# De-Rosa/PPO-BipedalWalker

Measured on NVIDIA B200. Metric: walker env-steps/sec (SAT physics step), higher is better.
Workload: dtype f32

## Files before the change

### ppo-bipedalwalker_b200/csrc/physics_lanes.cu

```cuda
#include <cstdio>
#include <cstdlib>
#include "physics.cuh"
#include "physics_math.cuh"

#ifndef WB_SAT_UNROLL
#define WB_SAT_UNROLL 6
#endif
#ifndef WB_BODY_SLOT
#define WB_BODY_SLOT 0
#endif

namespace wb {
namespace pl {
constexpr int kSatUnroll = WB_SAT_UNROLL;

constexpr unsigned kFull = 0xFFFFFFFFu;

#ifdef WB_PHASE_PROFILE
__device__ unsigned long long g_prof[24];
__device__ __forceinline__ long long prof_clock() {
  long long t;
  asm volatile("mov.u64 %0, %%clock64;" : "=l"(t)::"memory");
  return t;
}
__device__ long long g_prof_sat_scratch;
#endif


__constant__ Material c_materials[WB_MAX_MATERIALS];
__constant__ float c_init_state[kStateFloats];
__constant__ FloorConst c_floor;

enum { LLL = 0, LLU = 1, BODY = 2, RLL = 3, RLU = 4, FLOOR = 5 };

constexpr int kV2Cen = 30;
constexpr int kV2Vel = 35;
constexpr int kV2Count = 40;
constexpr int kFOmega = 0;
constexpr int kFAngle = 5;
constexpr int kFCount = 10;

__device__ __forceinline__ int nverts(int b) { return b == BODY ? 5 : 6; }

template <int L_, int E_>
struct Env {
  static constexpr int L = L_;
  static constexpr int E = E_;
  float2* v2;
  float* f;
  const FloorConst* fl;
  int sub;
  int gsub;
  int gshift;
  int col;
  bool live;
  int flags;
  float im_w;
  float ii_pole;
  float e_ww, mu_ww, e_wf, mu_wf;
};

template <class EV> __device__ __forceinline__ float2& V2(const EV& e, int slot) { return e.v2[slot * EV::E]; }
template <class EV> __device__ __forceinline__ float& F1(const EV& e, int slot) { return e.f[slot * EV::E]; }
template <class EV> __device__ __forceinline__ float inv_inertia(const EV& e, int b) { return b == BODY ? 0.0003f : e.ii_pole; }
template <class EV> __device__ __forceinline__ void set_materials(EV& e, const Material& mw, const Material& mf) {
  e.im_w = mw.inverse_mass;
  e.ii_pole = fmul(0.001f, mw.inverse_mass);
  e.e_ww = net_max(mw.restitution, mw.restitution);
  e.mu_ww = net_min(mw.friction, mw.friction);
  e.e_wf = net_max(mw.restitution, mf.restitution);
  e.mu_wf = net_min(mw.friction, mf.friction);
}
template <int L> __device__ __forceinline__ void lanes_sync() { if (L > 1) __syncwarp(); }
template <class EV, int G> __device__ __forceinline__ bool group_any(const EV& e, bool pred) {
  if (EV::L == 1) return pred;
  const unsigned b = __ballot_sync(kFull, pred);
  return ((b >> e.gshift) & ((1u << G) - 1u)) != 0u;
}

struct BodyDyn {
  float2 c, v;
  float w, im, ii;
};

template <class EV> __device__ __forceinline__ BodyDyn load_dyn(const EV& e, int b) {
  BodyDyn d;
  d.c = V2(e, kV2Cen + b);
  d.v = V2(e, kV2Vel + b);
  d.w = F1(e, kFOmega + b);
  d.im = e.im_w;
  d.ii = inv_inertia(e, b);
  return d;
}
template <class EV> __device__ __forceinline__ BodyDyn floor_dyn(const EV& e) {
  BodyDyn d;
  d.c = e.fl->cen;
  d.v = mk2(0.0f, 0.0f);
  d.w = 0.0f;
  d.im = 0.0f;
  d.ii = 0.0f;
  return d;
}
template <class EV> __device__ __forceinline__ void store_dyn(const EV& e, int b, const BodyDyn& d) {
  V2(e, kV2Vel + b) = d.v;
  F1(e, kFOmega + b) = d.w;
}

__device__ __forceinline__ void calculate_impulse(const BodyDyn& A, const BodyDyn& B, float2 contact, float force, float2 n,
                                                  float2& rA, float2& rB, float& impulse) {
  rA = vsub(contact, A.c);
  const float2 perpA = mk2(-rA.y, rA.x);
  const float kA = vdot(n, perpA);
  rB = vsub(contact, B.c);
  const float2 perpB = mk2(-rB.y, rB.x);
  const float kB = vdot(n, perpB);
  const float2 va = vadd(A.v, vmul(perpA, A.w));
  const float2 vb = vadd(B.v, vmul(perpB, B.w));
  const float2 vrel = vsub(vb, va);
  const float vn = vdot(vrel, n);
  const float j = fmul(-force, vn);
  const float2 k = mk2(kA, kB);
  const float2 kki = vmul2_nosum(vmul2_nosum(k, k), mk2(A.ii, B.ii));
  const float denom = fadd(fadd(fadd(A.im, B.im), kki.x), kki.y);
  impulse = fdiv(j, denom);
}

__device__ __forceinline__ void apply_impulses(BodyDyn& A, BodyDyn& B, float2 n, float impulse, float2 rA, float2 rB) {
  const float2 J = vmul(n, impulse);
  const float2 velA = vsub(A.v, vmul(J, A.im));
  const float2 velB = vadd(B.v, vmul(J, B.im));
  const float2 perpA = mk2(-rA.y, rA.x);
  const float wA = fsub(A.w, fmul(vdot(perpA, J), A.ii));
  const float2 perpB = mk2(-rB.y, rB.x);
  const float wB = fadd(B.w, fmul(vdot(perpB, J), B.ii));
  A.v = velA;
  B.v = velB;
  A.w = wA;
  B.w = wB;
}

template <class EV, int G>
__device__ __forceinline__ void move_bodies(const EV& e, bool on, int A, float2 dA, bool moveB, int B, float2 dB) {
#pragma unroll
  for (int it0 = 0; it0 < 14; it0 += G) {
    const int it = it0 + e.gsub;
    const bool second = it >= 7;
    const int k = second ? it - 7 : it;
    const int b = second ? B : A;
    if (on && it < 14 && (!second || moveB)) {
      const int slot = (k < 6) ? b * 6 + k : kV2Cen + b;
      V2(e, slot) = vadd(V2(e, slot), second ? dB : dA);
    }
  }
}

template <class EV, bool TRACE, int G = EV::L>
__device__ __forceinline__ void joint_step(const EV& e, int A, int ia, int B, int ib, wb_joint_trace* tr) {
  const bool leader = (G == EV::L) ? e.sub == 0 : e.gsub == 0;
  const float2 pA = V2(e, A * 6 + ia);
  const float2 pB = V2(e, B * 6 + ib);
  float2 ab = vsub(pB, pA);
  const float depth = fsqrt(vdot(ab, ab));
  if (TRACE) {
    if (tr && e.live && leader) {
      tr->active = !(depth < 0.1f);
      tr->depth = depth;
    }
  }
  const bool active = e.live && !(depth < 0.1f);
  if (!__any_sync(kFull, active)) return;
  ab = vnormalize_fast(ab);
  const float2 dA = vhalf(vmul(ab, depth));
  const float2 dB = vhalf(vmul(vneg(ab), depth));
  BodyDyn X = load_dyn(e, B);
  BodyDyn Y = load_dyn(e, A);
  lanes_sync<EV::L>();
  move_bodies<EV, G>(e, active, A, dA, true, B, dB);
  X.c = vadd(X.c, dB);
// ... 463 lines not shown
            rec.c1y = c1.y;
          }
        }
      }
      const float2 dA = FLOORB ? vmul(normal, depth) : vhalf(vmul(normal, depth));
      const float2 dB = FLOORB ? mk2(0.f, 0.f) : vhalf(vmul(vneg(normal), depth));
      lanes_sync<EV::L>();
      move_bodies<EV, G>(e, colliding, A, dA, !FLOORB, B, dB);
      X.c = vadd(X.c, dA);
      if (!FLOORB) Y.c = vadd(Y.c, dB);
      if (G == 1) {
        if (ncp > 0) resolve_impulses(X, Y, ncp, c0, c1, normal, FLOORB ? e.e_wf : e.e_ww, FLOORB ? e.mu_wf : e.mu_ww);
      } else {
        resolve_impulses_split(X, Y, ncp, c0, c1, normal, FLOORB ? e.e_wf : e.e_ww, FLOORB ? e.mu_wf : e.mu_ww, (e.gsub & 1) != 0);
      }
      if (ncp > 0 && colliding && e.gsub == 0) {
        store_dyn(e, A, X);
        if (!FLOORB) store_dyn(e, B, Y);
      }
      lanes_sync<EV::L>();
    }
  }
  if (TRACE) {
    if (tr && want && e.gsub == 0) *tr = rec;
  }
#ifdef WB_PHASE_PROFILE
  const unsigned prof_want = __ballot_sync(kFull, want), prof_coll = __ballot_sync(kFull, colliding);
  if (!TRACE && (threadIdx.x & 31) == 0) {
    const long long rp_t2 = prof_clock();
    const int k = FLOORB ? 1 : 0;
    atomicAdd(&g_prof[8 + 4 * k + 0], (unsigned long long)(rp_t1 - rp_t0));
    atomicAdd(&g_prof[8 + 4 * k + 1], (unsigned long long)(rp_t2 - rp_t1));
    atomicAdd(&g_prof[8 + 4 * k + 2], 1ull);
    atomicAdd(&g_prof[8 + 4 * k + 3], (unsigned long long)__popc(prof_want) | ((unsigned long long)__popc(prof_coll) << 32));
  }
#endif
}


template <class EV, int R>
__device__ __forceinline__ void integrate_step(const EV& e, bool on, int b, int q, int nq, float dt, float2 (&P)[R]) {
  float2 v = V2(e, kV2Vel + b);
  v = vadd(v, vmul(mk2(0.0f, 980.0f), dt));
  const float2 d = vmul(v, dt);
  const float w = F1(e, kFOmega + b);
  const float theta = fmul(w, dt);
  float ang = fadd(F1(e, kFAngle + b), theta);
  const float PI_F = 3.14159274f, TAU_F = 6.28318548f;
  if (ang > PI_F) ang = fsub(ang, TAU_F);
  else if (ang < -PI_F) ang = fadd(ang, TAU_F);
  float m11, m12;
  rotz(theta, m11, m12);
  const float2 cen = vadd(V2(e, kV2Cen + b), d);
  lanes_sync<EV::L>();
#pragma unroll
  for (int r = 0; r < R; r++) {
    const int i = r * nq + q;
    P[r] = mk2(0.0f, 0.0f);
    if (i < 6 && on) {
      float2 p = vadd(V2(e, b * 6 + i), d);
      p = vsub(p, cen);
      const float2 t = vrotate(p, m11, m12);
      P[r] = vadd(t, cen);
      V2(e, b * 6 + i) = P[r];
    }
  }
  if (q == 0 && on) {
    V2(e, kV2Cen + b) = cen;
    V2(e, kV2Vel + b) = v;
    F1(e, kFAngle + b) = ang;
  }
  lanes_sync<EV::L>();
}

template <class EV, int G, bool TRACE>
__device__ __forceinline__ void resolve_candidates(EV& e, bool on, int b, wb_pair_trace* tr_base) {
  const int slot = (0x75420 >> (4 * b)) & 0xF;
  const int partner = (0x34F01 >> (4 * b)) & 0xF;
  const bool floor_first = (e.flags & WB_FLAG_FLOOR_FIRST) != 0;
#pragma unroll 1
  for (int phase = 0; phase < 3; phase++) {
    if (phase == 1) {
      const bool want = on && b != BODY;
      if (__any_sync(kFull, want))
        resolve_pair<EV, G, TRACE, false>(e, want, b, b == BODY ? LLL : partner, (TRACE && tr_base) ? tr_base + slot + (floor_first ? 1 : 0) : nullptr);
    } else {
      const bool want = on && ((b == BODY) ? (phase == 0) : ((phase == 0) == floor_first));
      if (__any_sync(kFull, want))
        resolve_pair<EV, G, TRACE, true>(e, want, b, FLOOR, (TRACE && tr_base) ? tr_base + slot + ((b == BODY || floor_first) ? 0 : 1) : nullptr);
    }
  }
}

template <class EV, int G, bool TRACE>
__device__ __forceinline__ void body_step(EV& e, bool on, int b, float dt, wb_pair_trace* tr_base) {
  float2 P[(6 + G - 1) / G];
  integrate_step(e, on, b, e.gsub, G, dt, P);
  resolve_candidates<EV, G, TRACE>(e, on, b, tr_base);
}

template <class EV, int G, bool TRACE>
__device__ __forceinline__ void legs_sweep(EV& e, bool left, float dt, wb_pair_trace* tr_base) {
  static_assert(G >= 4, "two or more lanes per body in slot 0");
  constexpr int H = G / 2;
  constexpr int R = (6 + H - 1) / H;
  const int base = e.gshift - (left ? 0 : G);
#pragma unroll 1
  for (int k = 0; k < 2; k++) {
    const bool body_lane = k == 0 && left && e.gsub >= H;
    const int seg = left ? (k == 0 ? LLL : LLU) : (k == 0 ? RLL : RLU);
    float2 P[R];
    integrate_step(e, e.live, body_lane ? BODY : seg, body_lane ? e.gsub - H : e.gsub, (k == 0 && left) ? H : G, dt, P);
    if (k == 0) {
      float2 Q[6];
#pragma unroll
      for (int i = 0; i < 6; i++) {
        Q[i].x = __shfl_sync(kFull, P[i / H].x, base + H + i % H);
        Q[i].y = __shfl_sync(kFull, P[i / H].y, base + H + i % H);
      }
      float2 mn, mx;
      aabb6(Q, mn, mx);
      const unsigned hits = __ballot_sync(kFull, body_lane && e.live && aabb_hit(mn, mx, e.fl->bb_min, e.fl->bb_max));
      const bool body_hit = ((hits >> base) & ((1u << G) - 1u)) != 0u;
      if (body_hit) e.flags |= 1 << BODY;
      wb_pair_trace* tr = (TRACE && tr_base) ? tr_base + 4 : nullptr;
      if (TRACE) {
        if (tr && e.live && left && e.gsub == 0 && !body_hit) *tr = pair_trace_no_sat(FLOOR, false);
      }
      if (hits != 0u) resolve_pair<EV, G, TRACE, true, -1, true>(e, left && body_hit, left ? BODY : RLL, FLOOR, tr);
    }
    resolve_candidates<EV, G, TRACE>(e, e.live, seg, tr_base);
  }
}

template <class EV>
__device__ __forceinline__ void store_observation(const EV& e, float* dst) {
  const float2 j0 = V2(e, BODY * 6 + 1), j2 = V2(e, LLU * 6 + 2), j3 = V2(e, RLU * 6 + 2), bv = V2(e, kV2Vel + BODY);
  float4* d4 = reinterpret_cast<float4*>(dst);
  d4[0] = make_float4(fdiv(j0.x, 900.0f), fdiv(j0.y, 500.0f), fdiv(j2.x, 900.0f), fdiv(j2.y, 500.0f));
  d4[1] = make_float4(fdiv(j3.x, 900.0f), fdiv(j3.y, 500.0f), fdiv(bv.x, 60.0f), fdiv(bv.y, 60.0f));
  d4[2] = make_float4(F1(e, kFAngle + LLL), F1(e, kFAngle + LLU), F1(e, kFAngle + RLL), F1(e, kFAngle + RLU));
}

template <int E>
__device__ __forceinline__ int record_word(int f) {
  if (f < 58) {
    const int vtx = f >> 1, slot = vtx + (vtx >= 17 ? 1 : 0);
    return slot * E * 2 + (f & 1);
  }
  if (f < 78) return (kV2Cen + ((f - 58) >> 1)) * E * 2 + (f & 1);
  return kV2Count * E * 2 + (f - 78) * E;
}

template <int L, int LEGS, bool TRACE>
__global__ void __launch_bounds__(32, (L <= 4 || L == 16) ? 16 : 8) physics_lanes_kernel(const PhysicsParams p) {
  static_assert(LEGS == 1 || (LEGS == 2 && L >= 2), "the leg split needs at least two lanes per environment");
  constexpr int E = 32 / L;
  __shared__ __align__(16) float s_state[(kV2Count * 2 + kFCount) * E];
  __shared__ FloorConst s_floor;
  const int lane = threadIdx.x;
  const int env0 = blockIdx.x * E;

  for (int w = lane; w < (int)(sizeof(FloorConst) / 4); w += 32)
    reinterpret_cast<uint32_t*>(&s_floor)[w] = reinterpret_cast<const uint32_t*>(&c_floor)[w];
  for (int idx = lane; idx < 88 * E; idx += 32) {
    int f, c;
    if (idx < 78 * E) {
      const int slot = idx / (2 * E), r = idx % (2 * E);
      c = r >> 1;
      f = 2 * slot + (r & 1);
    } else {
      f = 78 + (idx - 78 * E) / E;
      c = idx % E;
    }
    const int env = env0 + c;
    const float v = (env < p.n) ? p.state[state_index(f, env, p.n_pad)] : c_init_state[f];
    s_state[record_word<E>(f) + (f < 78 ? 2 * c : c)] = v;
  }
  __syncwarp();

  using EV = Env<L, E>;
  EV e;
  const int col = lane / L;
  const int env = env0 + col;
  e.v2 = reinterpret_cast<float2*>(s_state) + col;
  e.f = s_state + kV2Count * E * 2 + col;
  e.fl = &s_floor;
  e.sub = lane % L;
  e.gsub = e.sub;
  e.gshift = col * L;
  e.live = env < p.n;
  const int envc = e.live ? env : 0;
  if (e.sub == 0) V2(e, BODY * 6 + 5) = V2(e, BODY * 6);
  float* torque_rows = p.state + (size_t)88 * p.n_pad + envc;

  e.flags = p.flags[envc];
  int steps = p.steps[envc];
  {
    const Material mw = c_materials[p.walker_mat[envc]];
    const Material mf = c_materials[p.floor_mat[envc]];
    set_materials(e, mw, mf);
  }
  float2 pos = mk2(p.pos[envc], p.pos[p.n_pad + envc]);
  __syncwarp();

  auto write_initial_record = [&](bool on) {
    if (!__any_sync(kFull, on)) return;
    __syncwarp();
    if (on && e.sub == 0) {
#pragma unroll 1
      for (int f = 0; f < 88; f++) s_state[record_word<E>(f) + (f < 78 ? 2 * col : col)] = c_init_state[f];
      V2(e, BODY * 6 + 5) = V2(e, BODY * 6);
      for (int k = 0; k < 4; k++) torque_rows[(size_t)k * p.n_pad] = c_init_state[88 + k];
    }
    __syncwarp();
  };

  if (p.phases & kPhaseResetMasked) {
    const bool on = e.live && (p.reset_mask == nullptr || p.reset_mask[envc]);
    write_initial_record(on);
    if (on) {
      e.flags = (p.phases & kPhaseFirstEpisode) ? 0 : WB_FLAG_FLOOR_FIRST;
      steps = 0;
      pos = V2(e, kV2Cen + BODY);
    }
  }
  if (p.phases & kPhaseIncSteps) steps++;

  if (p.phases & kPhaseTakeActions) {
    if (e.live && e.sub == 0) {
      const float4 a4 = *reinterpret_cast<const float4*>(p.actions + (size_t)env * 4);
      const float act[4] = {a4.x, a4.y, a4.z, a4.w};
#pragma unroll
      for (int k = 0; k < 4; k++) {
        float a = act[k];
        if (a >= 1.0f) a = 1.0f;
        else if (a <= -1.0f) a = -1.0f;
        const float change = fsub(a, torque_rows[(size_t)k * p.n_pad]);
        torque_rows[(size_t)k * p.n_pad] = a;
        const int bodyB = (k == 0) ? LLU : (k == 1) ? RLU : (k == 2) ? LLL : RLL;
        F1(e, kFOmega + bodyB) = fadd(F1(e, kFOmega + bodyB), fmul(change, 5.0f));
      }
    }
    __syncwarp();
  }

  if (p.phases & kPhaseStepObjects) {
    const float dt = fdiv(p.dt, (float)p.iterations);
#pragma unroll 1
    for (int it = 0; it < p.iterations; it++) {
      wb_joint_trace* jt = nullptr;
      wb_pair_trace* pt = nullptr;
      if (TRACE) {
        if (p.joint_trace) jt = p.joint_trace + ((size_t)envc * p.iterations + it) * 4;
        if (p.pair_trace) pt = p.pair_trace + ((size_t)envc * p.iterations + it) * WB_PAIR_SLOTS;
      }
      if (LEGS == 1) {
#pragma unroll 1
        for (int k = 0; k < 4; k++) {
          const int A = (0x4122 >> (4 * k)) & 0xF, B = (0x3041 >> (4 * k)) & 0xF;
          joint_step<EV, TRACE>(e, A, k < 2 ? 1 : 2, B, k < 2 ? 4 : 3, jt ? jt + k : nullptr);
        }
      } else {
        constexpr int G = L / LEGS;
        joint_step<EV, TRACE>(e, BODY, 1, LLU, 4, jt ? jt + 0 : nullptr);
        const int leg = e.sub / G;
        e.gsub = e.sub % G;
        e.gshift = col * L + leg * G;
        const bool left = leg == 0;
        joint_step<EV, TRACE, G>(e, left ? LLU : BODY, left ? 2 : 1, left ? LLL : RLU, left ? 3 : 4, jt ? jt + (left ? 2 : 1) : nullptr);
        e.gsub = e.sub;
        e.gshift = col * L;
        joint_step<EV, TRACE>(e, RLU, 2, RLL, 3, jt ? jt + 3 : nullptr);
      }
      if (LEGS == 1) {
#pragma unroll 1
        for (int b = 0; b < 5; b++) body_step<EV, L, TRACE>(e, e.live, b, dt, pt);
      } else {
        constexpr int G = L / LEGS;
        const int leg = e.sub / G;
        e.gsub = e.sub % G;
        e.gshift = col * L + leg * G;
        if constexpr (G >= 4 && !WB_BODY_SLOT) {
          legs_sweep<EV, G, TRACE>(e, leg == 0, dt, pt);
        } else {
#pragma unroll 1
          for (int k = 0; k < 3; k++) {
            const bool on = e.live && (leg == 0 || k < 2);
            body_step<EV, G, TRACE>(e, on, leg == 0 ? k : (k < 2 ? RLL + k : RLU), dt, pt);
          }
        }
        e.gsub = e.sub;
        e.gshift = col * L;
      }
    }
    if (LEGS == 2) e.flags |= __shfl_xor_sync(kFull, e.flags, L / LEGS);
  }

  if (p.phases & kPhaseObserve) {
    const float2 prev = pos;
    pos = V2(e, kV2Cen + BODY);
    if (e.flags & ((1 << BODY) | (1 << LLU) | (1 << RLU))) e.flags |= WB_FLAG_TERMINAL;
    const float dx = fsub(pos.x, prev.x);
    const float h = fdiv(V2(e, BODY * 6 + 1).y, 500.0f);
    float r = 0.0f;
    r = fadd(r, (dx > 0.0f && h < 1.6f) ? dx : 0.0f);
    r = fsub(r, (h > 1.65f) ? -0.1f : 0.0f);
    bool terminal = false;
    if ((e.flags & WB_FLAG_TERMINAL) || steps > p.max_timesteps) {
      if (e.flags & WB_FLAG_TERMINAL) r = fsub(r, 40.0f);
      terminal = true;
    }
    if (pos.x > 900.0f) {
      r = fadd(r, 80.0f);
      terminal = true;
    }
    const bool reset_now = e.live && terminal && (p.phases & kPhaseAutoReset);
    write_initial_record(reset_now);
    if (reset_now) {
      e.flags = WB_FLAG_FLOOR_FIRST;
      steps = 0;
      pos = V2(e, kV2Cen + BODY);
    }
    if (e.live && e.sub == 0) {
      store_observation(e, p.obs + (size_t)env * WB_OBS);
      p.reward[env] = r;
      p.done[env] = terminal ? 1 : 0;
    }
  } else if (p.phases & kPhaseObsOnly) {
    if (e.live && e.sub == 0) store_observation(e, p.obs + (size_t)env * WB_OBS);
  }

  if (e.live && e.sub == 0) {
    p.flags[env] = e.flags;
    p.steps[env] = steps;
    p.pos[env] = pos.x;
    p.pos[p.n_pad + env] = pos.y;
  }
  __syncwarp();
  for (int idx = lane; idx < 88 * E; idx += 32) {
    int f, c;
    if (idx < 78 * E) {
      const int slot = idx / (2 * E), r = idx % (2 * E);
      c = r >> 1;
      f = 2 * slot + (r & 1);
    } else {
      f = 78 + (idx - 78 * E) / E;
      c = idx % E;
    }
    if (env0 + c < p.n) p.state[state_index(f, env0 + c, p.n_pad)] = s_state[record_word<E>(f) + (f < 78 ? 2 * c : c)];
  }
}

__global__ void rcp_sqrt_check_kernel(uint32_t first, uint64_t count, unsigned long long* mismatches, uint32_t* first_bad) {
  const uint64_t stride = (uint64_t)gridDim.x * blockDim.x;
  unsigned long long bad = 0;
  for (uint64_t i = (uint64_t)blockIdx.x * blockDim.x + threadIdx.x; i < count; i += stride) {
    const uint32_t bits = first + (uint32_t)i;
    const float s = __uint_as_float(bits);
    const uint32_t a = __float_as_uint(rcp_sqrt_rn(s));
    const uint32_t b = __float_as_uint(__frcp_rn(__fsqrt_rn(s)));
    const bool both_nan = ((a & 0x7FFFFFFFu) > 0x7F800000u) && ((b & 0x7FFFFFFFu) > 0x7F800000u);
    if (a != b && !both_nan) {
      bad++;
      atomicMin(first_bad, bits);
    }
  }
  if (bad) atomicAdd(mismatches, bad);
}

__global__ void rotz_debug_kernel(const float* radians, int n, int mode, float* c_out, float* s_out) {
  const int i = blockIdx.x * blockDim.x + threadIdx.x;
  if (i >= n) return;
  float c, s;
  if (mode == 1) {
    sincos_dd_small((double)radians[i], c, s);
  } else if (mode == 2) {
    double sd, cd;
    sincos((double)radians[i], &sd, &cd);
    c = (float)cd;
    s = (float)sd;
  } else {
    rotz(radians[i], c, s);
  }
  c_out[i] = c;
  s_out[i] = s;
}

template <int L, int LEGS>
static cudaError_t launch_l(const PhysicsParams& p, bool trace, cudaStream_t stream) {
  constexpr int E = 32 / L;
  const int grid = (p.n + E - 1) / E;
  if (trace)
    physics_lanes_kernel<L, LEGS, true><<<grid, 32, 0, stream>>>(p);
  else
    physics_lanes_kernel<L, LEGS, false><<<grid, 32, 0, stream>>>(p);
  return cudaGetLastError();
}

}

namespace bulk {
__device__ __forceinline__ uint32_t smem_u32(const void* p) { return (uint32_t)__cvta_generic_to_shared(p); }
__device__ __forceinline__ void mbar_init(unsigned long long* bar, uint32_t count) {
  asm volatile("mbarrier.init.shared::cta.b64 [%0], %1;" ::"r"(smem_u32(bar)), "r"(count) : "memory");
}
__device__ __forceinline__ void fence_mbar_init() { asm volatile("fence.mbarrier_init.release.cluster;" ::: "memory"); }
__device__ __forceinline__ void mbar_expect_tx(unsigned long long* bar, uint32_t bytes) {
  asm volatile("mbarrier.arrive.expect_tx.shared::cta.b64 _, [%0], %1;" ::"r"(smem_u32(bar)), "r"(bytes) : "memory");
}
__device__ __forceinline__ void mbar_wait(unsigned long long* bar, uint32_t parity) {
  uint32_t ok = 0;
  while (!ok) {
    asm volatile(
        "{\n\t"
        ".reg .pred p;\n\t"
        "mbarrier.try_wait.parity.shared::cta.b64 p, [%1], %2;\n\t"
        "selp.b32 %0, 1, 0, p;\n\t"
        "}"
        : "=r"(ok)
        : "r"(smem_u32(bar)), "r"(parity)
        : "memory");
  }
}
__device__ __forceinline__ void load(void* smem_dst, const void* gmem_src, uint32_t bytes, unsigned long long* bar) {
  asm volatile("cp.async.bulk.shared::cluster.global.mbarrier::complete_tx::bytes [%0], [%1], %2, [%3];" ::"r"(smem_u32(smem_dst)),
               "l"(gmem_src), "r"(bytes), "r"(smem_u32(bar))
               : "memory");
}
__device__ __forceinline__ void store(void* gmem_dst, const void* smem_src, uint32_t bytes) {
  asm volatile("cp.async.bulk.global.shared::cta.bulk_group [%0], [%1], %2;" ::"l"(gmem_dst), "r"(smem_u32(smem_src)), "r"(bytes) : "memory");
}
__device__ __forceinline__ void fence_proxy_async() { asm volatile("fence.proxy.async.shared::cta;" ::: "memory"); }
__device__ __forceinline__ void commit_and_wait_reads() {
  asm volatile("cp.async.bulk.commit_group;" ::: "memory");
  asm volatile("cp.async.bulk.wait_group.read 0;" ::: "memory");
}
}

namespace pc {
using namespace pl;

#ifdef WB_PHASE_PROFILE
#define WB_PROF_DECL long long prof_t = prof_clock(); unsigned long long prof_acc[4] = {0, 0, 0, 0}; unsigned long long prof_items = 0, prof_rounds = 0
#define WB_PROF_MARK(k) do { const long long now_ = prof_clock(); prof_acc[k] += (unsigned long long)(now_ - prof_t); prof_t = now_; } while (0)
#else
#define WB_PROF_DECL
#define WB_PROF_MARK(k)
#endif

template <int kE>
struct Shared {
  float state[(kV2Count * 2 + kFCount) * kE];
  Material mtab[WB_MAX_MATERIALS];
  unsigned char wmat[kE], fmat[kE];
  FloorConst floor;
  unsigned char axis[4 * kE];
  unsigned short queue[3 * kE];
  unsigned char jq[4 * kE];
  int count[2];
  unsigned long long stage_bar;
#ifdef WB_PHASE_PROFILE
  long long prof_arrive[2][2][32];
#endif
};
extern __shared__ __align__(16) unsigned char smem_pc[];
template <int kE> __device__ __forceinline__ Shared<kE>& shm() { return *reinterpret_cast<Shared<kE>*>(smem_pc); }

template <int kE> __device__ __forceinline__ void scope_sync() {
  if (kE == 32) __syncwarp(); else __syncthreads();
}
template <int kE> __device__ __forceinline__ bool scope_any(bool pred) {
  if (kE == 32) return __any_sync(kFull, pred) != 0;
  return __syncthreads_or(pred) != 0;
}

template <int kE>
__device__ __forceinline__ void env_for_column(Env<1, kE>& e, Shared<kE>& S, int col, bool live) {
  e.v2 = reinterpret_cast<float2*>(S.state) + col;
  e.f = S.state + kV2Count * kE * 2 + col;
  e.fl = &S.floor;
  e.sub = 0;
  e.gsub = 0;
  e.gshift = 0;
  e.live = live;
  e.flags = 0;
  set_materials(e, S.mtab[S.wmat[col]], S.mtab[S.fmat[col]]);
}

template <int kE>
__device__ __forceinline__ void push(Shared<kE>& S, int parity, bool want, int item) {
  const unsigned m = __ballot_sync(kFull, want);
  if (m == 0) return;
  const int lane = threadIdx.x & 31;
  int base = 0;
  if (lane == 0) base = atomicAdd(&S.count[parity], __popc(m));
  base = __shfl_sync(kFull, base, 0);
  if (want) S.queue[base + __popc(m & ((1u << lane) - 1u))] = (unsigned short)item;
}

__device__ __forceinline__ int pair_slot(int b) { return b == LLL ? 0 : b == LLU ? 1 : b == RLL ? 2 : 3; }
__device__ __forceinline__ int partner_of(int b) { return (0x34F01 >> (4 * b)) & 0xF; }

template <int kE>
// ... 481 lines not shown
        if (body_pending) integrate_body<kE>(tid, BODY, dt);
#endif
        if (any_first) {
#if WB_FUSED_FLOOR_TEST
          const bool f0 = floor_first && hit0, f1 = floor_first && hit1;
#else
          const bool f0 = floor_first && floor_pair_needs_work<kE>(tid, b0), f1 = floor_first && floor_pair_needs_work<kE>(tid, b1);
#endif
          e.flags |= (f0 ? 1 << b0 : 0) | (f1 ? 1 << b1 : 0);
          if (WB_F1_INWARP && ph == 1) {
            warp_floor_items<kE>(f0, b0, f1, b1);
          } else {
            push(S, parity, f0, tid | (b0 << 10));
            push(S, parity, f1, tid | (b1 << 10));
            if (body_pending) {
#if WB_FUSED_FLOOR_TEST
              const bool fb = hitb;
#else
              const bool fb = floor_pair_needs_work<kE>(tid, BODY);
#endif
              if (fb) e.flags |= 1 << BODY;
              push(S, parity, fb, tid | (BODY << 10));
              body_pending = false;
            }
            round([&] { drain<kItemFloor, kE>(parity); });
          }
        }
        push(S, parity, pole_pair_needs_work<kE>(tid, b0, partner_of(b0)), tid | (b0 << 10));
        push(S, parity, pole_pair_needs_work<kE>(tid, b1, partner_of(b1)), tid | (b1 << 10));
        round([&] { drain<kItemPole, kE>(parity); });
        if (any_last) {
          const bool f0 = !floor_first && floor_pair_needs_work<kE>(tid, b0), f1 = !floor_first && floor_pair_needs_work<kE>(tid, b1);
          e.flags |= (f0 ? 1 << b0 : 0) | (f1 ? 1 << b1 : 0);
          push(S, parity, f0, tid | (b0 << 10));
          push(S, parity, f1, tid | (b1 << 10));
          if (body_pending) {
            const bool fb = floor_pair_needs_work<kE>(tid, BODY);
            if (fb) e.flags |= 1 << BODY;
            push(S, parity, fb, tid | (BODY << 10));
            body_pending = false;
          }
          round([&] { drain<kItemFloor, kE>(parity); });
        }
      }
    }
#ifdef WB_PHASE_PROFILE
    if ((tid & 31) == 0) {
      for (int k = 0; k < 4; k++) atomicAdd(&g_prof[k], prof_acc[k]);
      atomicAdd(&g_prof[4], 1ull);
      if (tid == 0) {
        atomicAdd(&g_prof[5], prof_items);
        atomicAdd(&g_prof[6], prof_rounds);
      }
    }
#endif
  }

  if (p.phases & kPhaseObserve) {
    const float2 prev = pos;
    pos = V2(e, kV2Cen + BODY);
    if (e.flags & ((1 << BODY) | (1 << LLU) | (1 << RLU))) e.flags |= WB_FLAG_TERMINAL;
    const float dx = fsub(pos.x, prev.x);
    const float h = fdiv(V2(e, BODY * 6 + 1).y, 500.0f);
    float r = 0.0f;
    r = fadd(r, (dx > 0.0f && h < 1.6f) ? dx : 0.0f);
    r = fsub(r, (h > 1.65f) ? -0.1f : 0.0f);
    bool terminal = false;
    if ((e.flags & WB_FLAG_TERMINAL) || steps > p.max_timesteps) {
      if (e.flags & WB_FLAG_TERMINAL) r = fsub(r, 40.0f);
      terminal = true;
    }
    if (pos.x > 900.0f) {
      r = fadd(r, 80.0f);
      terminal = true;
    }
    if (live && terminal && (p.phases & kPhaseAutoReset)) {
      write_initial_record();
      e.flags = WB_FLAG_FLOOR_FIRST;
      steps = 0;
      pos = V2(e, kV2Cen + BODY);
    }
    if (live) {
      store_observation(e, p.obs + (size_t)env * WB_OBS);
      p.reward[env] = r;
      p.done[env] = terminal ? 1 : 0;
    }
  } else if (p.phases & kPhaseObsOnly) {
    if (live) store_observation(e, p.obs + (size_t)env * WB_OBS);
  }

  if (live) {
    p.flags[env] = e.flags;
    p.steps[env] = steps;
    p.pos[env] = pos.x;
    p.pos[p.n_pad + env] = pos.y;
    if (p.axis_cache != nullptr)
      p.axis_cache[env] = (uint32_t)S.axis[tid] | ((uint32_t)S.axis[kE + tid] << 8) | ((uint32_t)S.axis[2 * kE + tid] << 16) |
                          ((uint32_t)S.axis[3 * kE + tid] << 24);
    if (!kBulk) {
#pragma unroll 8
      for (int f = 0; f < 88; f++) p.state[state_index(f, env, p.n_pad)] = S.state[record_word<kE>(f) + (f < 78 ? 2 * tid : tid)];
    }
  }
  if (kBulk) {
    bulk::fence_proxy_async();
    scope_sync<kE>();
    if (tid == 0) {
#pragma unroll 1
      for (int s2 = 0; s2 < kStateSlots2; s2++) {
        const int col_slot = s2 < 17 ? s2 : (s2 < 29 ? s2 + 1 : (s2 < 34 ? kV2Cen + (s2 - 29) : kV2Vel + (s2 - 34)));
        bulk::store(p.state + ((size_t)s2 * p.n_pad + env0) * 2, S.state + (size_t)col_slot * kE * 2, kE * 8);
      }
#pragma unroll 1
      for (int r = 0; r < 10; r++)
        bulk::store(p.state + (size_t)(78 + r) * p.n_pad + env0, S.state + (size_t)kV2Count * kE * 2 + (size_t)r * kE, kE * 4);
      bulk::commit_and_wait_reads();
    }
  }
}

template <int kE>
static cudaError_t launch_compact(const PhysicsParams& p, cudaStream_t stream) {
  static bool configured[64] = {};
  int dev = 0;
  cudaGetDevice(&dev);
  if (dev < 0 || dev >= 64 || !configured[dev]) {
    cudaError_t e = cudaFuncSetAttribute(physics_compact_kernel<kE>, cudaFuncAttributeMaxDynamicSharedMemorySize, (int)sizeof(Shared<kE>));
    if (e != cudaSuccess) return e;
    e = cudaFuncSetAttribute(physics_compact_kernel<kE>, cudaFuncAttributePreferredSharedMemoryCarveout, cudaSharedmemCarveoutMaxShared);
    if (e != cudaSuccess) return e;
    if (getenv("WB_DEBUG_OCCUPANCY")) {
      int nb = 0;
      cudaOccupancyMaxActiveBlocksPerMultiprocessor(&nb, physics_compact_kernel<kE>, kE, sizeof(Shared<kE>));
      fprintf(stderr, "physics_compact_kernel<%d>: %d CTAs/SM, %zu B shared per CTA\n", kE, nb, sizeof(Shared<kE>));
    }
    if (dev >= 0 && dev < 64) configured[dev] = true;
  }
  physics_compact_kernel<kE><<<(p.n + kE - 1) / kE, kE, sizeof(Shared<kE>), stream>>>(p);
  return cudaGetLastError();
}

}

#ifdef WB_PHASE_PROFILE
extern "C" int wb_prof_read(unsigned long long* out24, int reset) {
  cudaDeviceSynchronize();
  if (cudaMemcpyFromSymbol(out24, pl::g_prof, sizeof(unsigned long long) * 24) != cudaSuccess) return 1;
  if (reset) {
    unsigned long long z[24] = {};
    cudaMemcpyToSymbol(pl::g_prof, z, sizeof(z));
  }
  return 0;
}
#endif

cudaError_t upload_materials(const Material* table, int count) {
  return cudaMemcpyToSymbol(pl::c_materials, table, sizeof(Material) * count);
}

cudaError_t upload_scene_constants(const float* init_state92, const FloorConst* floor) {
  cudaError_t e = cudaMemcpyToSymbol(pl::c_init_state, init_state92, sizeof(float) * kStateFloats);
  if (e != cudaSuccess) return e;
  return cudaMemcpyToSymbol(pl::c_floor, floor, sizeof(FloorConst));
}

bool physics_lanes_supported(int variant) {
  switch (variant) {
    case 1: case 2: case 4: case 8: case 16: case 32: case 104: case 108: case 116: case 1001: case 1002: case 1003: case 1004: case 1005: return true;
    default: return false;
  }
}

cudaError_t launch_physics(const PhysicsParams& p, int variant, bool trace, cudaStream_t stream) {
  switch (variant) {
    case 1: return pl::launch_l<1, 1>(p, trace, stream);
    case 2: return pl::launch_l<2, 2>(p, trace, stream);
    case 4: return pl::launch_l<4, 2>(p, trace, stream);
    case 8: return pl::launch_l<8, 2>(p, trace, stream);
    case 16: return pl::launch_l<16, 2>(p, trace, stream);
    case 32: return pl::launch_l<32, 2>(p, trace, stream);
    case 104: return pl::launch_l<4, 1>(p, trace, stream);
    case 108: return pl::launch_l<8, 1>(p, trace, stream);
    case 116: return pl::launch_l<16, 1>(p, trace, stream);
    case 1001: return trace ? pl::launch_l<1, 1>(p, true, stream) : pc::launch_compact<256>(p, stream);
    case 1002: return trace ? pl::launch_l<1, 1>(p, true, stream) : pc::launch_compact<32>(p, stream);
    case 1003: return trace ? pl::launch_l<1, 1>(p, true, stream) : pc::launch_compact<128>(p, stream);
    case 1004: return trace ? pl::launch_l<1, 1>(p, true, stream) : pc::launch_compact<192>(p, stream);
    case 1005: return trace ? pl::launch_l<1, 1>(p, true, stream) : pc::launch_compact<160>(p, stream);
    default: return cudaErrorInvalidValue;
  }
}

cudaError_t launch_rcp_sqrt_check(uint32_t first, uint64_t count, unsigned long long* mismatches_dev, uint32_t* first_bad_dev,
                                  cudaStream_t stream) {
  pl::rcp_sqrt_check_kernel<<<148 * 8, 256, 0, stream>>>(first, count, mismatches_dev, first_bad_dev);
  return cudaGetLastError();
}

cudaError_t launch_rotz_debug(const float* radians, int n, int mode, float* c_out, float* s_out, cudaStream_t stream) {
  pl::rotz_debug_kernel<<<(n + 255) / 256, 256, 0, stream>>>(radians, n, mode, c_out, s_out);
  return cudaGetLastError();
}

}
```

Baseline: 11.96 million.

## Stage walker state and per-env inputs with vectorized cp.async, vectorize writeback

Replaces the scalar per-float state load loop with vectorized cp.async copies into shared memory, and issues async copies of flags, steps, pos, material bytes, torques and actions alongside it, so all global loads are in flight together before a single wait. The writeback uses float2/float4 stores when the whole CTA's environments are live. Dead columns are filled with initial state separately, and the reset path writes the initial record in parallel across lanes. It also adds optional per-phase clock profiling under a compile flag. It relies on alignment assumptions about n_pad and env0 for the vector accesses, and reads material indices as 4-byte words.

```diff
diff --git a/ppo-bipedalwalker_b200/csrc/physics_lanes.cu b/ppo-bipedalwalker_b200/csrc/physics_lanes.cu
--- a/ppo-bipedalwalker_b200/csrc/physics_lanes.cu
+++ b/ppo-bipedalwalker_b200/csrc/physics_lanes.cu
@@ -1,5 +1,6 @@
 #include <cstdio>
 #include <cstdlib>
+#include <type_traits>
 #include "physics.cuh"
 #include "physics_math.cuh"
 
@@ -24,6 +25,8 @@
   return t;
 }
 __device__ long long g_prof_sat_scratch;
+constexpr int kLanesProfCtas = 1 << 16;
+__device__ unsigned long long g_lanes_prof[3 * kLanesProfCtas];
 #endif
 
 
@@ -793,32 +796,57 @@
   return kV2Count * E * 2 + (f - 78) * E;
 }
 
+struct __align__(16) WalkerInputs {
+  float4 actions;
+  float torque[4];
+  float2 pos;
+  int32_t flags, steps;
+  uint32_t mat_words[2];
+};
+
+template <int V> struct FloatVec;
+template <> struct FloatVec<1> { using T = float; };
+template <> struct FloatVec<2> { using T = float2; };
+template <> struct FloatVec<4> { using T = float4; };
+
+template <int E, class F>
+__device__ __forceinline__ void for_record_pieces(int lane, int env0, int n_pad, F&& fn) {
+  constexpr int VA = 2 * E < 4 ? 2 * E : 4, PA = 2 * E / VA, NA = kStateSlots2 * PA;
+  constexpr int VB = E < 4 ? E : 4, PB = E / VB, NB = kFCount * PB;
+#pragma unroll
+  for (int j = 0; j < (NA + 31) / 32; j++) {
+    const int i = j * 32 + lane, s2 = i / PA, k = i % PA;
+    if (NA % 32 == 0 || i < NA)
+      fn(((size_t)s2 * n_pad + env0) * 2 + k * VA, (s2 + (s2 >= 17 ? 1 : 0)) * 2 * E + k * VA, k * VA / 2, 2,
+         std::integral_constant<int, VA>());
+  }
+#pragma unroll
+  for (int j = 0; j < (NB + 31) / 32; j++) {
+    const int i = j * 32 + lane, r = i / PB, k = i % PB;
+    if (NB % 32 == 0 || i < NB)
+      fn((size_t)(78 + r) * n_pad + env0 + k * VB, kV2Count * 2 * E + r * E + k * VB, k * VB, 1, std::integral_constant<int, VB>());
+  }
+}
+
+template <int B>
+__device__ __forceinline__ void cp_async(float* smem, const float* gmem) {
+  asm volatile("cp.async.ca.shared.global [%0], [%1], %2;" ::"r"((uint32_t)__cvta_generic_to_shared(smem)), "l"(gmem), "n"(B)
+               : "memory");
+}
+__device__ __forceinline__ void cp_async_wait_all() { asm volatile("cp.async.wait_all;" ::: "memory"); }
+
 template <int L, int LEGS, bool TRACE>
 __global__ void __launch_bounds__(32, (L <= 4 || L == 16) ? 16 : 8) physics_lanes_kernel(const PhysicsParams p) {
   static_assert(LEGS == 1 || (LEGS == 2 && L >= 2), "the leg split needs at least two lanes per environment");
   constexpr int E = 32 / L;
   __shared__ __align__(16) float s_state[(kV2Count * 2 + kFCount) * E];
   __shared__ FloorConst s_floor;
+  __shared__ WalkerInputs s_in[E];
   const int lane = threadIdx.x;
   const int env0 = blockIdx.x * E;
-
-  for (int w = lane; w < (int)(sizeof(FloorConst) / 4); w += 32)
-    reinterpret_cast<uint32_t*>(&s_floor)[w] = reinterpret_cast<const uint32_t*>(&c_floor)[w];
-  for (int idx = lane; idx < 88 * E; idx += 32) {
-    int f, c;
-    if (idx < 78 * E) {
-      const int slot = idx / (2 * E), r = idx % (2 * E);
-      c = r >> 1;
-      f = 2 * slot + (r & 1);
-    } else {
-      f = 78 + (idx - 78 * E) / E;
-      c = idx % E;
-    }
-    const int env = env0 + c;
-    const float v = (env < p.n) ? p.state[state_index(f, env, p.n_pad)] : c_init_state[f];
-    s_state[record_word<E>(f) + (f < 78 ? 2 * c : c)] = v;
-  }
-  __syncwarp();
+#ifdef WB_PHASE_PROFILE
+  const long long t_entry = prof_clock();
+#endif
 
   using EV = Env<L, E>;
   EV e;
@@ -832,27 +860,62 @@
   e.gshift = col * L;
   e.live = env < p.n;
   const int envc = e.live ? env : 0;
+  float* torque_rows = p.state + (size_t)88 * p.n_pad + envc;
+
+  for_record_pieces<E>(lane, env0, p.n_pad, [&](size_t g, int s, int, int, auto v) {
+    cp_async<decltype(v)::value * 4>(s_state + s, p.state + g);
+  });
+  WalkerInputs& in = s_in[col];
+  if (e.sub == 0) {
+    cp_async<4>(reinterpret_cast<float*>(&in.flags), reinterpret_cast<const float*>(p.flags + envc));
+    cp_async<4>(reinterpret_cast<float*>(&in.steps), reinterpret_cast<const float*>(p.steps + envc));
+    cp_async<4>(&in.pos.x, p.pos + envc);
+    cp_async<4>(&in.pos.y, p.pos + p.n_pad + envc);
+    cp_async<4>(reinterpret_cast<float*>(&in.mat_words[0]), reinterpret_cast<const float*>(p.walker_mat + (envc & ~3)));
+    cp_async<4>(reinterpret_cast<float*>(&in.mat_words[1]), reinterpret_cast<const float*>(p.floor_mat + (envc & ~3)));
+    if (p.phases & kPhaseTakeActions) {
+#pragma unroll
+      for (int k = 0; k < 4; k++) cp_async<4>(&in.torque[k], torque_rows + (size_t)k * p.n_pad);
+      if (e.live) cp_async<16>(reinterpret_cast<float*>(&in.actions), p.actions + (size_t)env * 4);
+    }
+  }
+  constexpr int kFloorWords = sizeof(FloorConst) / 4;
+#pragma unroll
+  for (int j = 0; j < (kFloorWords + 31) / 32; j++) {
+    const int w = j * 32 + lane;
+    if (w < kFloorWords) reinterpret_cast<uint32_t*>(&s_floor)[w] = reinterpret_cast<const uint32_t*>(&c_floor)[w];
+  }
+  cp_async_wait_all();
+  __syncwarp();
+  e.flags = in.flags;
+  int steps = in.steps;
+  float2 pos = in.pos;
+  {
+    const int byte = 8 * (envc & 3);
+    set_materials(e, c_materials[(in.mat_words[0] >> byte) & 0xFFu], c_materials[(in.mat_words[1] >> byte) & 0xFFu]);
+  }
+
+  auto write_initial_column = [&]() {
+#pragma unroll 1
+    for (int j = 0; j < (88 + L - 1) / L; j++) {
+      const int f = j * L + e.sub;
+      if (88 % L == 0 || f < 88) s_state[record_word<E>(f) + (f < 78 ? 2 * col : col)] = c_init_state[f];
+    }
+  };
+  if (!e.live) write_initial_column();
+  __syncwarp();
   if (e.sub == 0) V2(e, BODY * 6 + 5) = V2(e, BODY * 6);
-  float* torque_rows = p.state + (size_t)88 * p.n_pad + envc;
-
-  e.flags = p.flags[envc];
-  int steps = p.steps[envc];
-  {
-    const Material mw = c_materials[p.walker_mat[envc]];
-    const Material mf = c_materials[p.floor_mat[envc]];
-    set_materials(e, mw, mf);
-  }
-  float2 pos = mk2(p.pos[envc], p.pos[p.n_pad + envc]);
   __syncwarp();
 
   auto write_initial_record = [&](bool on) {
     if (!__any_sync(kFull, on)) return;
     __syncwarp();
+    if (on) write_initial_column();
+    __syncwarp();
     if (on && e.sub == 0) {
-#pragma unroll 1
-      for (int f = 0; f < 88; f++) s_state[record_word<E>(f) + (f < 78 ? 2 * col : col)] = c_init_state[f];
       V2(e, BODY * 6 + 5) = V2(e, BODY * 6);
-      for (int k = 0; k < 4; k++) torque_rows[(size_t)k * p.n_pad] = c_init_state[88 + k];
+#pragma unroll
+      for (int k = 0; k < 4; k++) torque_rows[(size_t)k * p.n_pad] = in.torque[k] = c_init_state[88 + k];
     }
     __syncwarp();
   };
@@ -870,14 +933,13 @@
 
   if (p.phases & kPhaseTakeActions) {
     if (e.live && e.sub == 0) {
-      const float4 a4 = *reinterpret_cast<const float4*>(p.actions + (size_t)env * 4);
-      const float act[4] = {a4.x, a4.y, a4.z, a4.w};
+      const float act[4] = {in.actions.x, in.actions.y, in.actions.z, in.actions.w};
 #pragma unroll
       for (int k = 0; k < 4; k++) {
         float a = act[k];
         if (a >= 1.0f) a = 1.0f;
         else if (a <= -1.0f) a = -1.0f;
-        const float change = fsub(a, torque_rows[(size_t)k * p.n_pad]);
+        const float change = fsub(a, in.torque[k]);
         torque_rows[(size_t)k * p.n_pad] = a;
         const int bodyB = (k == 0) ? LLU : (k == 1) ? RLU : (k == 2) ? LLL : RLL;
         F1(e, kFOmega + bodyB) = fadd(F1(e, kFOmega + bodyB), fmul(change, 5.0f));
@@ -886,6 +948,9 @@
     __syncwarp();
   }
 
+#ifdef WB_PHASE_PROFILE
+  const long long t_substeps = prof_clock();
+#endif
   if (p.phases & kPhaseStepObjects) {
     const float dt = fdiv(p.dt, (float)p.iterations);
 #pragma unroll 1
@@ -937,6 +1002,9 @@
     }
     if (LEGS == 2) e.flags |= __shfl_xor_sync(kFull, e.flags, L / LEGS);
   }
+#ifdef WB_PHASE_PROFILE
+  const long long t_observe = prof_clock();
+#endif
 
   if (p.phases & kPhaseObserve) {
     const float2 prev = pos;
@@ -979,18 +1047,26 @@
     p.pos[p.n_pad + env] = pos.y;
   }
   __syncwarp();
-  for (int idx = lane; idx < 88 * E; idx += 32) {
-    int f, c;
-    if (idx < 78 * E) {
-      const int slot = idx / (2 * E), r = idx % (2 * E);
-      c = r >> 1;
-      f = 2 * slot + (r & 1);
+  const bool all_live = env0 + E <= p.n;
+  for_record_pieces<E>(lane, env0, p.n_pad, [&](size_t g, int s, int c0, int per_col, auto v) {
+    constexpr int V = decltype(v)::value;
+    using T = typename FloatVec<V>::T;
+    if (all_live) {
+      *reinterpret_cast<T*>(p.state + g) = *reinterpret_cast<const T*>(s_state + s);
     } else {
-      f = 78 + (idx - 78 * E) / E;
-      c = idx % E;
-    }
-    if (env0 + c < p.n) p.state[state_index(f, env0 + c, p.n_pad)] = s_state[record_word<E>(f) + (f < 78 ? 2 * c : c)];
-  }
+#pragma unroll
+      for (int j = 0; j < V; j++)
+        if (env0 + c0 + j / per_col < p.n) p.state[g + j] = s_state[s + j];
+    }
+  });
+#ifdef WB_PHASE_PROFILE
+  if (lane == 0 && blockIdx.x < kLanesProfCtas) {
+    const long long t_end = prof_clock();
+    g_lanes_prof[3 * blockIdx.x + 0] = t_substeps - t_entry;
+    g_lanes_prof[3 * blockIdx.x + 1] = t_observe - t_substeps;
+    g_lanes_prof[3 * blockIdx.x + 2] = t_end - t_observe;
+  }
+#endif
 }
 
 __global__ void rcp_sqrt_check_kernel(uint32_t first, uint64_t count, unsigned long long* mismatches, uint32_t* first_bad) {
@@ -1778,6 +1854,11 @@
   }
   return 0;
 }
+extern "C" int wb_lanes_prof_read(unsigned long long* out, int ctas) {
+  if (ctas < 0 || ctas > pl::kLanesProfCtas) return 1;
+  cudaDeviceSynchronize();
+  return cudaMemcpyFromSymbol(out, pl::g_lanes_prof, sizeof(unsigned long long) * 3 * ctas) != cudaSuccess;
+}
 #endif
 
 cudaError_t upload_materials(const Material* table, int count) {
```

After: 12.41 million, median of 6. 1.04x the previous value.
